# tiiuae/MLAdversarialObjectDetection

Measured on AMD Instinct MI355X. Metric: patch-opt images/sec (EffDet-D0 512px fwd+bwd), higher is better.
Workload: dtype f32; 1 GPU; C2: EfficientDet-D0 patch attack 512x512, 16 images/GPU, bn=local; global_batch=16, image_size=512, placement=injected, parallelism=dp1

## Files before the change

### mladversarialobjectdetection_amd/build.py

```python
import os
import subprocess
import sys

HERE = os.path.dirname(os.path.abspath(__file__))


def build(jobs: int = 8, verbose: bool = False) -> str:
    csrc = os.path.join(HERE, "csrc")
    env = dict(os.environ)
    cmd = ["make", "-C", csrc, f"-j{min(jobs, 16)}"]
    r = subprocess.run(cmd, env=env, stdout=subprocess.PIPE, stderr=subprocess.STDOUT, text=True)
    if verbose or r.returncode != 0:
        sys.stdout.write(r.stdout)
    if r.returncode != 0:
        raise RuntimeError("libphx build failed")
    kern = os.path.join(os.path.dirname(HERE), "tests", "kernels")
    if os.path.isfile(os.path.join(kern, "Makefile")):
        r = subprocess.run(["make", "-C", kern, f"-j{min(jobs, 16)}"], env=env, stdout=subprocess.PIPE,
                           stderr=subprocess.STDOUT, text=True)
        if verbose or r.returncode != 0:
            sys.stdout.write(r.stdout)
        if r.returncode != 0:
            raise RuntimeError("tests/kernels build failed")
    return os.path.join(HERE, "libphx.so")


if __name__ == "__main__":
    print(build(verbose=True))
```

### mladversarialobjectdetection_amd/csrc/api.cpp

```cpp
#include "ctx.hpp"

namespace {

std::string json_escape(const std::string& s) {
  std::string o;
  for (char c : s) {
    if (c == '"' || c == '\\') o.push_back('\\');
    o.push_back(c);
  }
  return o;
}

std::vector<float> make_anchors(const ModelConfig& mc) {
  std::vector<int> fs{mc.image_size};
  int f = mc.image_size;
  for (int l = 1; l <= mc.max_level; ++l) {
    f = (f - 1) / 2 + 1;
    fs.push_back(f);
  }
  std::vector<float> out;
  for (int level = mc.min_level; level <= mc.max_level; ++level) {
    const double stride = (double)fs[0] / (double)fs[level];
    struct C { double base_x, base_y, ax, ay; };
    std::vector<C> cs;
// ... 688 lines not shown
  PHX_CATCH(ctx)
}

int phx_debug_tap(phx_ctx* ctx, const char* op_name, int which, float* out, size_t nfloats, void* stream) {
  if (!ctx || !op_name || !out || ctx->execs.empty()) return PHX_EINVAL;
  PHX_TRY(ctx)
  if (!ctx->last) throw std::logic_error("no step has run");
  Exec& E = *ctx->last;
  for (size_t i = 0; i < E.prog.ops.size(); ++i) {
    const Op& op = E.prog.ops[i];
    if (op.name != op_name) continue;
    const int t = (op.t == OP_BN && which == 0) ? op.in[0] : op.out;
    if (nfloats != E.prog.tensors[t].numel())
      throw std::invalid_argument("tap: size mismatch (the tensor has " + std::to_string(E.prog.tensors[t].numel()) +
                                  " elements)");
    if (which == 0 && op.t == OP_FUSE && E.fuse_folded[i])
      throw std::invalid_argument("tap: this fuse is computed on load by its depthwise conv, never stored");
    if (which == 1 && op.t == OP_DW && E.sepb[i])
      throw std::invalid_argument("tap: this depthwise output's gradient is formed in LDS by the fused "
                                  "separable-conv backward, never stored (PHX_SEPB=0 keeps it)");
    if (which == 0 && op.t == OP_DW && E.sep[i])
      throw std::invalid_argument("tap: this depthwise output feeds the fused separable conv's registers only, "
                                  "never stored (PHX_SEP=0 at victim creation keeps it)");
    const float* src = which == 0 ? E.tptr(t, nullptr) : E.gptr(op.out);
    if (!src) throw std::invalid_argument("tap: no gradient for this tensor");
    if (which == 0 && E.tbf(t)) launch_bf16_to_f32(src, out, (long)nfloats, (hipStream_t)stream);
    else PHX_HIP(hipMemcpyAsync(out, src, nfloats * 4, hipMemcpyDeviceToDevice, (hipStream_t)stream));
    return PHX_OK;
  }
  throw std::invalid_argument(std::string("tap: no op named ") + op_name);
  PHX_CATCH(ctx)
}

int phx_debug_tensor(phx_ctx* ctx, int tag, int op_index, int which, void* out, size_t nbytes, void* stream) {
  if (!ctx || !out || ctx->execs.empty()) return PHX_EINVAL;
  PHX_TRY(ctx)
  if (!ctx->last) throw std::logic_error("no step has run");
  Exec* E = nullptr;
  for (auto& e : ctx->execs)
    if (e->B == ctx->last->B && e->tag == tag) E = e.get();
  if (!E) throw std::invalid_argument("tensor: no executor with this tag");
  if (op_index < 0 || op_index >= (int)E->prog.ops.size() || which < 0 || which > 2)
    throw std::invalid_argument("tensor: bad op index / which");
  const Op& op = E->prog.ops[op_index];
  const int t = which == 0 ? op.out : op.in[which - 1];
  if (t < 0 || t == E->prog.input) throw std::invalid_argument("tensor: no such arena tensor");
// ... 64 lines not shown
```

### mladversarialobjectdetection_amd/csrc/dw_stage.hpp

```cpp
#pragma once
#include <type_traits>

#include "common.hpp"

namespace phx {

__device__ __forceinline__ bool dw_block_map(int L, int per, int ncg, int nwork, int* tile,
                                             int* cg) {
  const int w = (L & 7) * per + (L >> 3);
  if ((L >> 3) >= per || w >= nwork) return false;
  *tile = w / ncg;
  *cg = w - *tile * ncg;
  return true;
}

template <bool BF>
struct StageInX {
  using Raw = float4;
  InX v;
  Chan4 k;
  bool f;
  __device__ __forceinline__ void init(const InX& x, int c) {
    v = x;
    f = x.mu != nullptr;
// ... 68 lines not shown
  }
  __device__ __forceinline__ Raw zero() const {
    return Raw{make_float4(0.f, 0.f, 0.f, 0.f), make_float4(0.f, 0.f, 0.f, 0.f)};
  }
  __device__ __forceinline__ Raw load(long e) const {
    Raw r;
    r.d = *reinterpret_cast<const float4*>(g.da + e);
    if (g.y) r.y = ald4<BF>(g.y, e);
    return r;
  }
  __device__ __forceinline__ float4 finish(const Raw& r) const {
    return g.y ? gx_apply4(g, k, r.d, r.y) : r.d;
  }
  static constexpr bool kActT = true;
  __device__ __forceinline__ int act() const { return g.y ? g.act : 0; }
  template <int ACT>
  __device__ __forceinline__ float4 finish_t(const Raw& r) const {
    GradX c = g;
    c.act = ACT;
    return g.y ? gx_apply4(c, k, r.d, r.y) : r.d;
  }
};

__device__ __forceinline__ void fma4(float4& a, const float4& x, const float4& w) {
  a.x = fmaf(x.x, w.x, a.x);
  a.y = fmaf(x.y, w.y, a.y);
  a.z = fmaf(x.z, w.z, a.z);
  a.w = fmaf(x.w, w.w, a.w);
}

}
```

### mladversarialobjectdetection_amd/csrc/exec.cpp

```cpp
#include "ctx.hpp"

constexpr size_t kMaxExecs = 4;

namespace {

void alloc_exec(Exec& E, int A) {
  const Program& P = E.prog;
  const int B = E.B;
  E.act = E.alloc<float>(E.abf ? (P.act_floats + 1) / 2 : P.act_floats);
  E.grad = E.alloc<float>(E.tag != 0 ? 1 : P.grad_floats);
  E.slot_a.assign(P.n_slots, nullptr);
  E.slot_b.assign(P.n_slots, nullptr);
  E.slot_c.assign(P.n_slots, nullptr);
  E.slot_d.assign(P.n_slots, nullptr);
  E.slot_e.assign(P.n_slots, nullptr);
  for (const Op& op : P.ops) {
    const Tensor& ti = P.tensors[op.in[0]];
    if (op.t == OP_BN) {
      E.slot_a[op.slot] = E.alloc<float>(ti.c);
      E.slot_b[op.slot] = E.alloc<float>(ti.c);
      E.slot_c[op.slot] = E.alloc<float>(ti.c);
      E.slot_d[op.slot] = E.alloc<float>(ti.c);
      E.slot_e[op.slot] = E.alloc<float>(ti.c);
      PHX_HIP(hipMemset(E.slot_d[op.slot], 0, ti.c * sizeof(float)));
// ... 201 lines not shown
  if (op.t == OP_BN) {
    ck_note(E, nm + " mean", E.slot_a[op.slot], ti.c * 4, s);
    ck_note(E, nm + " rstd", E.slot_b[op.slot], ti.c * 4, s);
    ck_note(E, nm + " scale", E.slot_c[op.slot], ti.c * 4, s);
  } else if (op.t == OP_SE) {
    ck_note(E, nm + " excite", E.slot_c[op.slot], (size_t)E.B * ti.c * 4, s);
  } else {
    const Tensor& to = P.tensors[op.out];
    ck_note(E, nm + " out", E.tptr(op.out, nullptr), to.numel() * (E.tbf(op.out) ? 2 : 4), s);
  }
}

void ck_post(Exec& E, int pass, hipStream_t s) {
  const size_t n0 = E.ck_names.size();
  for (size_t i = 0; i < E.prog.ops.size(); ++i) ck_fwd(E, (int)i, pass, s);
  for (size_t k = n0; k < E.ck_names.size(); ++k) E.ck_names[k] = "post " + E.ck_names[k];
}

static void ck_bwd(Exec& E, int i, hipStream_t s) {
  if (!E.ck_on) return;
  const Program& P = E.prog;
  const Op& op = P.ops[i];
  const std::string nm = "b " + std::to_string(i) + " " + op.name;
  if (op.t == OP_BN) {
    const int C = P.tensors[op.in[0]].c;
    ck_note(E, nm + " mdz", E.slot_d[op.slot], C * 4, s);
    ck_note(E, nm + " mdzx", E.slot_e[op.slot], C * 4, s);
    return;
  }
  for (int k = 0; k < op.nin; ++k)
    if (const float* g = E.gptr(op.in[k])) ck_note(E, nm + " d" + std::to_string(k), g, P.tensors[op.in[k]].numel() * 4, s);
}

static bool frozen_reuse_off() {
  return !env_on("PHX_FROZEN_REUSE");
}


static void sync_reduce_apply(phx_ctx* ctx, Exec& E, const BnFinSeg* segs, int n, int C, bool bwd, hipStream_t s) {
  if (!ctx->ar_fn) throw std::logic_error("bn=sync: no collective registered (phx_set_allreduce)");
  if (ctx->ar_fn(ctx->ar_user, E.sync_sums, (size_t)n * C * 3, s) != 0)
    throw std::runtime_error("bn=sync: the all-reduce callback failed");
  launch_bn_from_sums(segs, n, C, bwd, E.sync_sums, kBnEps, s);
}

static void sync_finalize(phx_ctx* ctx, Exec& E, const BnFinSeg* segs, int n, int C, bool bwd, hipStream_t s) {
// ... 503 lines not shown
  else
    for (size_t k = 0; k < zp.size(); ++k) PHX_HIP(hipMemsetAsync(zp[k], 0, zb[k], s));
  launch_cls_scatter(E.scores, E.keep, E.mraw, E.nties, E.dm, E.tptr(P.cls_out[0], input),
                     E.lev_dev, (int)E.lev.size(), ctx->A, E.B, ctx->mc.num_classes, na,
                     W + wpred, K, E.grad, E.dxoff_dev, s, E.tbf(P.cls_out[0]));
  for (int i = (int)P.ops.size() - 1; i >= 0; --i) {
    const Op& op = P.ops[i];
    if (!op.bwd) continue;
    if (op.t == OP_PW && is_cls_out(P, op.out)) continue;
    if (i > 0 && E.sepb[i - 1]) continue;
    if (E.grp_of[i] >= 0) {
      if (E.groups[E.grp_of[i]].back() == i) {
        if (E.sepb[i]) run_sep_bwd(ctx, E, i, input, s);
        else run_group_bwd(ctx, E, E.grp_of[i], input, s);
        for (int m : E.groups[E.grp_of[i]]) ck_bwd(E, m, s);
      }
      continue;
    }
    if (E.sepb[i]) {
      run_sep_bwd(ctx, E, i, input, s);
      ck_bwd(E, i, s);
      continue;
    }
    const Tensor& ti = P.tensors[op.in[0]];
    const Tensor& to = P.tensors[op.out];
    const float* dy = E.gptr(op.out);
    float* dx = E.gptr(op.in[0]);
    double fl = 0, by = 4.0 * (double)(ti.numel() + to.numel());
    const char* kind = "bwd_other";
    switch (op.t) {
      case OP_STEM: kind = "stem_bwd"; fl = 2.0 * to.numel() * 27; break;
      case OP_PW: kind = "gemm"; fl = 2.0 * ti.rows() * ti.c * to.c; by += 4.0 * ti.c * to.c; break;
      case OP_DW: kind = "dw_bwd"; fl = 2.0 * to.numel() * op.k * op.k; break;
      case OP_BN: kind = "bn_bwd_reduce"; by = 4.0 * 2.0 * ti.numel(); break;
      case OP_SE: kind = "se_bwd"; by = 4.0 * 3.0 * ti.numel(); break;
      default: break;
    }
    if (op.t == OP_PW || op.t == OP_DW) {
      const int bi = E.bn_consumer[op.out];
      if (bi >= 0 && P.ops[bi].bwd) by += 4.0 * (double)to.numel();
      if (op.acc[0]) by += 4.0 * (double)ti.numel();
    }
    GradSink gsk{};
    int gsk_in = -1;
    if (i > 0 && E.gfused_bn[i - 1]) {
      const Op& bn = P.ops[i - 1];
      gsk = GradSink{E.spart, P.tensors[bn.out].c, 0, E.tptr(bn.in[0], input), E.slot_a[bn.slot],
                     E.slot_b[bn.slot], E.slot_c[bn.slot], W + bn.beta, bn.act, E.tbf(bn.in[0])};
      gsk_in = op.in[0] == bn.out ? 0 : 1;
    }
    if (op.t == OP_BN && E.gfused_bn[i]) by = 8.0 * (double)E.gstat_P[i] * ti.c;
    if (skip_kind(std::string("b:") + kind, op.name)) continue;
    Scope scope(ctx, kind, fl, by, s, (prof_detail() || debug_sync()) ? op_tag(P, op, true) : std::string());
    int np = -1;
    switch (op.t) {
      case OP_STEM: {
        GradX g = gview(ctx, E, op.out, input);
        if (!op.acc[0] && stem_bwd_gx_supported(to.c)) {
          launch_stem_bwd_gx(g, W + op.w, E.owner, dx, ti.n, ti.h, ti.w, to.h, to.w, to.c, op.pad_t,
                             op.pad_l, s);
          break;
        }
        float* gy = E.gptr(op.out);
        if (g.y) launch_bn_bwd_apply2(g, gy, (long)to.rows(), to.c, s);
        launch_stem_bwd(g.y ? gy : g.da, W + op.w, dx, ti.n, ti.h, ti.w, to.h, to.w, to.c, op.pad_t, op.pad_l,
                        op.acc[0], s);
        break;
      }
      case OP_PW:
        np = launch_gemm_dgrad(gview(ctx, E, op.out, input), W + op.w, dx, (int)ti.rows(), ti.c, to.c,
                               op.acc[0], s, E.gpart, gsk, E.bf16);
        break;
      case OP_DW:
        np = launch_dw_bwd(gview(ctx, E, op.out, input), W + op.w, dx, ti.n, ti.h, ti.w, ti.c, to.h, to.w, op.k,
                           op.stride, op.pad_t, op.pad_l, op.acc[0], s, gsk);
        break;
      case OP_BN:
        if (op.acc[0]) throw std::runtime_error("BN input with several consumers");
        if (!frozen && E.gfused_bn[i] && ctx->bn_mode == PHX_BN_SYNC) {
          const BnFinSeg sg{E.spart + E.gstat_region[i] * E.sp_region, nullptr, E.gstat_P[i], (long)ti.rows(),
                            nullptr, nullptr, nullptr, nullptr, nullptr, nullptr, E.slot_d[op.slot], E.slot_e[op.slot]};
          sync_finalize(ctx, E, &sg, 1, ti.c, true, s);
        } else if (!frozen && E.gfused_bn[i] && skip_timing('b')) {
        } else if (!frozen && E.gfused_bn[i])
          launch_bn_bwd_finalize(E.spart + E.gstat_region[i] * E.sp_region, E.gstat_P[i], (long)ti.rows(),
                                 ti.c, E.slot_d[op.slot],
                                 E.slot_e[op.slot], s);
        else if (!frozen && ctx->bn_mode == PHX_BN_SYNC) {
          launch_bn_bwd_reduce_sums(dy, E.tptr(op.in[0], input), E.slot_a[op.slot], E.slot_b[op.slot], W + op.gamma,
                                    W + op.beta, (long)ti.rows(), ti.c, op.act, E.red, E.sync_sums, s,
                                    E.tbf(op.in[0]) != 0);
          const BnFinSeg sg{nullptr, nullptr, 0, (long)ti.rows(), nullptr, nullptr, nullptr, nullptr, nullptr, nullptr,
                            E.slot_d[op.slot], E.slot_e[op.slot]};
          sync_reduce_apply(ctx, E, &sg, 1, ti.c, true, s);
        }
        else if (!frozen)
          launch_bn_bwd_reduce(dy, E.tptr(op.in[0], input), E.slot_a[op.slot], E.slot_b[op.slot],
                               W + op.gamma, W + op.beta, (long)ti.rows(), ti.c, op.act, E.red,
                               E.slot_d[op.slot], E.slot_e[op.slot], s, E.tbf(op.in[0]) != 0);
        (void)dx;
        break;
      case OP_SE:
        np = launch_se_bwd(dy, view(ctx, E, op.in[0], input), dx, ti.n, ti.h * ti.w, ti.c, op.cse, W + op.w1,
                           W + op.b1, ctx->wt_of(op.w2), W + op.b2, op.act, E.slot_a[op.slot],
                           E.slot_b[op.slot], E.slot_c[op.slot], E.se_g, op.acc[0], s, E.red, gsk);
        break;
      case OP_ADD: {
        int n0 = 0, n1 = 0;
        if (dx == dy) {
          if (gsk_in == 0) n0 = launch_grad_sums(dy, (long)to.numel(), to.c, gsk, s);
        } else {
          n0 = launch_copy_grad(dy, dx, (long)to.numel(), op.acc[0], s, to.c,
                                gsk_in == 0 ? gsk : GradSink{}, drop_view(E, i));
        }
        if (E.gptr(op.in[1]) == dy) {
          if (gsk_in == 1) n1 = launch_grad_sums(dy, (long)to.numel(), to.c, gsk, s);
        } else {
          n1 = launch_copy_grad(dy, E.gptr(op.in[1]), (long)to.numel(), op.acc[1], s, to.c,
                                gsk_in == 1 ? gsk : GradSink{});
        }
        np = gsk_in == 0 ? n0 : n1;
        break;
      }
      case OP_MAXPOOL:
        launch_maxpool_bwd(E.pool_amax[i], dy, dx, ti.n, ti.h, ti.w, ti.c, to.h, to.w,
// ... 106 lines not shown
```

### mladversarialobjectdetection_amd/csrc/exec_plan.cpp

```cpp
#include "exec_plan.hpp"

#include <algorithm>
#include <map>
#include <stdexcept>

#include "env.hpp"
#include "phx.h"

namespace phx {

bool is_cls_out(const Program& P, int t) {
  return std::find(P.cls_out.begin(), P.cls_out.end(), t) != P.cls_out.end();
}

namespace {

bool grouping_enabled() {
  static const bool on = env_on("PHX_GROUP");
  return on;
}

bool group_uniform(const ExecPlan& E, const std::vector<int>& v) {
  const Program& P = E.prog;
  const Op& a = P.ops[v[0]];
// ... 264 lines not shown
      if (gd >= 0 && E.groups[gd][0] != (int)i) continue;
      const std::vector<int> mem = gd >= 0 ? E.groups[gd] : std::vector<int>{(int)i};
      bool ok = true;
      for (int di : mem) {
        const Op& d = P.ops[di];
        const Op& pw = P.ops[di + 1];
        const int bi = E.bn_consumer[pw.out];
        ok = ok && d.bwd && pw.bwd && !is_cls_out(P, pw.out) && bi >= 0 && P.ops[bi].bwd &&
             sep_bwd_supported(P.tensors[d.in[0]].c, P.tensors[pw.out].c, E.bf16 || E.abf);
        ok = ok && (di > 0 && E.gfused_bn[di - 1]) == (mem[0] > 0 && E.gfused_bn[mem[0] - 1]);
      }
      if (!ok) continue;
      for (int di : mem) {
        E.sepb[di] = 1;
        if (di > 0 && E.gfused_bn[di - 1]) {
          const Tensor& tm = P.tensors[P.ops[di].in[0]];
          const int np = sep_stat_partials(tm.n, tm.h, tm.w);
          E.gstat_P[di - 1] = np;
          sp_need = std::max(sp_need, (size_t)np * tm.c);
        }
      }
    }
  }
  E.nreg = E.groups.empty() ? 1 : kMaxSeg;
  E.sp_region = sp_need;
  E.sc_region = sc_need;
  for (const Op& op : P.ops) {
    if (op.t != OP_PW) continue;
    const Tensor& ti = P.tensors[op.in[0]];
    const Tensor& to = P.tensors[op.out];
    E.gp_need = std::max(E.gp_need, gemm_partial_floats((int)ti.rows(), to.c, ti.c, bf16));
    E.gp_need = std::max(E.gp_need, gemm_partial_floats((int)ti.rows(), ti.c, to.c, bf16));
  }
  const int nlev = (int)P.cls_out.size();
  int a0 = 0;
  for (int l = 0; l < nlev; ++l) {
    const Tensor& tc = P.tensors[P.cls_out[l]];
    const Tensor& tb = P.tensors[P.box_out[l]];
    LevelDesc d;
    d.cls_off = (long)tc.off - (long)P.tensors[P.cls_out[0]].off;
    d.box_off = (long)tb.off - (long)P.tensors[P.box_out[0]].off;
    d.h = tc.h;
    d.w = tc.w;
    d.anchor0 = a0;
    d.tile0 = E.ntiles;
    E.ntiles += pre_nms_tiles(tc.h, tc.w, na);
// ... 27 lines not shown
```

### mladversarialobjectdetection_amd/csrc/exec_plan.hpp

```cpp
#pragma once
#include <vector>

#include "common.hpp"
#include "kernels.hpp"
#include "model.hpp"
#include "post.hpp"

namespace phx {

struct ExecPlan {
  Program prog;
  int B = 0;
  int tag = 0;
  bool bf16 = false;
  bool abf = false;
  bool infer_plan = false;
  std::vector<int> se_of_tensor;
  std::vector<int> bn_of_tensor;
  std::vector<int> bn_consumer;
  std::vector<char> fused_bn;
  std::vector<char> gfused_bn;
  std::vector<int> gstat_P;
  std::vector<int> grp_of;
  std::vector<std::vector<int>> groups;
  std::vector<char> fuse_folded;
  std::vector<char> sep;
  std::vector<char> sepb;
  std::vector<int> drop_slot;
  std::vector<int> side_off;
  std::vector<MovEntry> mov;
  int n_mov = 0, mov_cmax = 1;
  std::vector<LevelDesc> lev;
  std::vector<long> dxoff;
  int ntiles = 0;
  int ndrop = 0;
  std::vector<int> drop_blocks;
  std::vector<float> drop_surv;
  EotDims ed{};
  size_t red_need = 1, coef_need = 1, seg_need = 1, gp_need = 1;
  size_t sp_region = 1, sc_region = 1, nreg = 1;
  size_t side_need = 2, sync_need = 0;
};

ExecPlan plan_exec(const ModelConfig& mc, int B, int tag, int bn_mode, bool bf16, int num_anchors);

ExecPlan plan_program(const Program& prog, int B, int tag, int bn_mode, bool bf16, int image_size, int na,
                      int num_anchors);

bool is_cls_out(const Program& P, int t);

// ... 2 lines not shown
```

### mladversarialobjectdetection_amd/csrc/kernels.hpp

```cpp
#pragma once
#include <hip/hip_runtime.h>
#include <hip/hip_ext.h>

#include <cstddef>
#include <cstdint>

#include "common.hpp"

namespace phx {

struct ExtTiming {
  hipEvent_t a = nullptr, b = nullptr;
  bool used = false;
};
ExtTiming*& ext_timing();
#define PHX_TLAUNCH(K, G, BL, SHM, S, ...)                                                              \
  do {                                                                                                 \
    if (::phx::ExtTiming* t_ = ::phx::ext_timing()) {                                                  \
      hipExtLaunchKernelGGL(K, G, BL, SHM, S, t_->used ? nullptr : t_->a, t_->b, 0, __VA_ARGS__);      \
      t_->used = true;                                                                                 \
    } else {                                                                                           \
      hipLaunchKernelGGL(K, G, BL, SHM, S, __VA_ARGS__);                                               \
    }                                                                                                  \
  } while (0)
// ... 49 lines not shown
int gemm_dgrad_gsink_partials(int M, int N, int K, bool bf16 = false);
bool gemm_fold_ok(int M, int N, int K, bool bf16);
struct GemmSeg {
  InX A;
  GradX G;
  const float* bias;
  float* C;
  int M;
  bool acc;
  StatSink sink;
  GradSink gsk;
};
bool gemm_group_ok(const int* M, int n, int N, int K, bool bf16 = false);
int gemm_group_run(int mode, const GemmSeg* segs, int n, const float* Bt, int N, int K, hipStream_t s,
                   bool bf16 = false, int* P_out = nullptr, long max_part_rows = -1);
int launch_dw_fwd(InX x, const float* w, float* y, int B, int H, int W, int C, int Ho,
                  int Wo, int k, int stride, int pt, int pl, hipStream_t s,
                  StatSink sink = StatSink{});
int dw_stat_partials(int B, int H, int W, int C, int Ho, int Wo, int k, int stride, int pt, int pl);
int launch_dw_bwd(GradX dy, const float* w, float* dx, int B, int H, int W, int C, int Ho,
                  int Wo, int k, int stride, int pt, int pl, bool acc, hipStream_t s,
                  GradSink gs = GradSink{});
int dw_bwd_partials(int B, int H, int W, int C, int Ho, int Wo, int k, int stride, int pt, int pl);
struct DwSeg {
  InX x;
  GradX gv;
  float* out;
  int H, W, Ho, Wo, pt, pl;
  bool acc;
  StatSink sink;
  GradSink gs;
};
void launch_dw_fwd_group(const DwSeg* segs, int n, int B, int C, const float* w, int k, int stride,
                         hipStream_t s, int* nps);
struct SepMember {
  InX x;
  FuseView f;
  bool fuse;
  float* y;
  int H, W;
  StatSink sink;
};
bool sep_supported(int C, int N, bool bf16);
int sep_stat_partials(int B, int H, int W);
void launch_sep_fwd(const SepMember* m, int n, int B, int C, int N, const float* wd, const float* bt,
                    const float* bias, hipStream_t s, int* nps);
// ... 64 lines not shown
void launch_bn_stats_sums(const float* y, long M, int C, double* part, double* sums, hipStream_t s, bool ybf);
void launch_bn_bwd_reduce_sums(const float* da, const float* y, const float* mean, const float* rstd,
                               const float* gamma, const float* beta, long M, int C, int act, double* part,
                               double* sums, hipStream_t s, bool ybf);
void launch_bn_bwd_finalize_group(const BnFinSeg* segs, int n, int C, hipStream_t s);
void launch_bn_frozen_stats(const float* mmean, const float* mvar, float* mean, float* rstd,
                            const float* gamma, float* sc, int C, float eps, hipStream_t s);
void launch_bn_apply(const float* y, const float* mean, const float* rstd, const float* gamma,
                     const float* beta, float* a, long M, int C, int act, hipStream_t s);
void launch_bn_bwd(const float* da, const float* y, const float* mean, const float* rstd,
                   const float* gamma, const float* beta, float* dy, long M, int C, int act,
                   bool frozen, bool acc, double* part, float* coef, hipStream_t s);
void launch_bn_bwd_apply2(GradX g, float* out, long M, int C, hipStream_t s);
void launch_bn_bwd_reduce(const float* da, const float* y, const float* mean, const float* rstd,
                          const float* gamma, const float* beta, long M, int C, int act,
                          double* part, float* mdz, float* mdzx, hipStream_t s, bool ybf = false);
void launch_se_fwd(InX x, float* y, int B, int HW, int C, int Cse, const float* w1,
                   const float* b1, const float* w2, const float* b2, int act, float* pool,
                   float* hidden, float* scale, hipStream_t s, double* scratch);
int launch_se_bwd(const float* dy, InX x, float* dx, int B, int HW, int C, int Cse,
                  const float* w1, const float* b1, const float* w2t, const float* b2, int act,
                  const float* pool, const float* hidden, const float* scale, float* gsum,
                  bool acc, hipStream_t s, double* scratch, GradSink gs = GradSink{});
int ew_gstats_partials(long seg_rows, int C, int nseg);
void launch_bn_bwd_finalize(const float2* part, int P, long M, int C, float* mdz, float* mdzx,
                            hipStream_t s);
size_t colred_scratch_doubles(long seg_rows, int C, int nseg);
struct RedPlanInfo {
  int tpr, rpi, cgroups, chunks, tpr_last, depth;
  long rpc;
};
RedPlanInfo red_plan_info(long seg_rows, int C, int nseg);
struct SePlanInfo {
  int s1, cs1, s2, cs2, fold_small, kg, jg;
};
SePlanInfo se_plan_info(int B, int C, int Cse, int chunks);
struct DropView {
  const float* keep = nullptr;
  float p = 1.f;
  long rows = 1;
};
void launch_drop_keep(const int* block, const float* p, int nd, int B, uint64_t seed, int64_t step,
                      int gimg0, int pass, float* keep, hipStream_t s);
void launch_bf16_to_f32(const float* src, float* dst, long n, hipStream_t s);
void launch_cksum(const void* p, size_t bytes, unsigned long long* out, hipStream_t s);
void launch_add(InX a, InX b, float* y, long n, int C, hipStream_t s, DropView dv = DropView{});
// ... 87 lines not shown
```

### mladversarialobjectdetection_amd/csrc/kernels_dw.hip

```cpp
#include <algorithm>
#include <cstdlib>
#include <stdexcept>
#include <type_traits>

#include "env.hpp"
#include "dw_stage.hpp"
#include "kernels.hpp"

namespace phx {

struct DwGeom {
  int H, W, C;
  int Ho, Wo;
  int pt, pl;
  int lcg;
  int otw, oth;
  int nrg;
  int rin, cin;
  int tiles_x, ntiles, ncg;
  int per;
};

template <class XV>
struct DwFwdSegT {
  XV x;
  float* y;
  DwGeom g;
  StatSink sink;
};
using DwFwdSeg = DwFwdSegT<InX>;
template <int NS, class XV = InX>
struct DwFwdGroup {
  DwFwdSegT<XV> s[NS];
  const float* w;
};
struct DwBwdSeg {
  GradX gv;
  float* dx;
  DwGeom g;
  int acc;
  GradSink gs;
};
template <int NS>
struct DwBwdGroup {
  DwBwdSeg s[NS];
  const float* w;
};

#ifndef PHX_DW_LDS_TAPS
#define PHX_DW_LDS_TAPS 2
#endif
template <int K>
struct Taps {
  static constexpr bool kLds = PHX_DW_LDS_TAPS == 2 || (PHX_DW_LDS_TAPS == 1 && K > 3);
  float4 r[kLds ? 1 : K * K];
  const float4* l;
  int cg, CG;
  __device__ __forceinline__ void stage(float4* wt, const float* w, int C, int cgi, int lcg) {
    if constexpr (kLds) {
      const int n = (K * K) << lcg;
      for (int e = threadIdx.x; e < n; e += 256) {
        const int t = e >> lcg, k = e & ((1 << lcg) - 1);
        wt[e] = *reinterpret_cast<const float4*>(w + (long)t * C + (((cgi << lcg) + k) << 2));
      }
// ... 190 lines not shown
  const int lane = threadIdx.x & 63, wave = threadIdx.x >> 6;
  s1 = dw_xor_sum(s1, lcg);
  s2 = dw_xor_sum(s2, lcg);
  if (lane < CG) {
    a_[wave][cg] = s1;
    b_[wave][cg] = s2;
  }
  __syncthreads();
  if (threadIdx.x < CG) {
    float4 t1 = a_[0][cg], t2 = b_[0][cg];
#pragma unroll
    for (int w = 1; w < 4; ++w) {
      const float4 u = a_[w][cg], v = b_[w][cg];
      t1.x += u.x; t1.y += u.y; t1.z += u.z; t1.w += u.w;
      t2.x += v.x; t2.y += v.y; t2.z += v.z; t2.w += v.w;
    }
    gsink_put(g, p, c + 0, t1.x, t2.x);
    gsink_put(g, p, c + 1, t1.y, t2.y);
    gsink_put(g, p, c + 2, t1.z, t2.z);
    gsink_put(g, p, c + 3, t1.w, t2.w);
  }
}

template <int K, int S, int RPT, bool GS, int NS, int SU = 4, bool YBF = false>
__global__ __launch_bounds__(256) void k_dw_bwd(DwBwdGroup<NS> grp) {
  const DwBwdSeg sg = pick_seg(grp.s, NS == 1 ? 0 : (int)blockIdx.y);
  const GradX& gv = sg.gv;
  const DwGeom& g = sg.g;
  const GradSink& gsk = sg.gs;
  const int acc_flag = sg.acc;
  const float* __restrict__ w = grp.w;
  float* __restrict__ dx = sg.dx;
  extern __shared__ float4 tile[];
  const int b = blockIdx.z;
  int tl, cgi;
  if (!dw_block_map(blockIdx.x, g.per, g.ncg, g.ntiles * g.ncg, &tl, &cgi)) return;
  const int CG = 1 << g.lcg;
  const int ty = tl / g.tiles_x, tx = tl - ty * g.tiles_x;
  const int iy0 = ty * g.oth, ix0 = tx * g.otw;
  const int cg = threadIdx.x & (CG - 1), q = threadIdx.x >> g.lcg;
  const int col = q % g.otw, rg = q / g.otw;
  const int c = (cgi * CG + cg) * 4;
  const int ay = iy0 + g.pt - (K - 1), ax = ix0 + g.pl - (K - 1);
  const int oy_lo = S == 1 ? ay : (ay >= 0 ? ay / S : -((-ay + S - 1) / S));
  const int ox_lo = S == 1 ? ax : (ax >= 0 ? ax / S : -((-ax + S - 1) / S));

  StageGradX<YBF> src;
  src.init(gv, c);
  float4* wt = tile + g.rin * g.cin * CG;
  Taps<K> wr;
  wr.stage(wt, w, g.C, cgi, g.lcg);
  dw_stage<StageGradX<YBF>, SU>(tile, src, b, g.Ho, g.Wo, g.C, oy_lo, ox_lo, c, g);
  __syncthreads();

  const int ix = ix0 + col;
  const int row0 = rg * RPT;
  const bool active = rg < g.nrg && ix < g.W && iy0 + row0 < g.H;
  if (!GS && !active) return;
  float4 acc[RPT];
#pragma unroll
  for (int r = 0; r < RPT; ++r) acc[r] = make_float4(0.f, 0.f, 0.f, 0.f);
  if (active) {
    wr.init(wt, w, g.C, c, cg, g.lcg);
    if constexpr (S == 1) {
      constexpr int NR = RPT + K - 1;
      const float4* base = tile + (row0 * g.cin + col) * CG + cg;
#pragma unroll
      for (int ir = 0; ir < NR; ++ir) {
#pragma unroll
        for (int jj = 0; jj < K; ++jj) {
          const float4 v = base[(ir * g.cin + jj) * CG];
#pragma unroll
          for (int r = 0; r < RPT; ++r) {
            const int ii = ir - r;
            if (ii >= 0 && ii < K) fma4(acc[r], v, wr((K - 1 - ii) * K + (K - 1 - jj)));
// ... 180 lines not shown
  if (dw_lds(grp.s[0].g, k) > 160 * 1024) throw std::runtime_error("dw: LDS window too large");
  dw_fwd_go<3, 1, 4, 1, FuseView>(grp, 1, B, false, s);
  PHX_LAUNCH_CHECK();
}

void launch_dw_fwd_group(const DwSeg* segs, int n, int B, int C, const float* w, int k, int stride,
                         hipStream_t s, int* nps) {
  if (C % 4) throw std::runtime_error("dw: C % 4 != 0");
  if (n < 1 || n > kMaxSeg) throw std::runtime_error("dw group: bad member count");
  const int rpt = dw_rpt_fwd(stride);
  DwFwdGroup<kMaxSeg> grp{};
  grp.w = w;
  const bool stats = segs[0].sink.part != nullptr;
  for (int i = 0; i < n; ++i) {
    const DwSeg& d = segs[i];
    if ((d.sink.part != nullptr) != stats) throw std::runtime_error("dw group: members differ in sinks");
    grp.s[i] = DwFwdSeg{d.x, d.out, dw_plan(d.H, d.W, C, d.Ho, d.Wo, d.pt, d.pl, k, stride, rpt, false), d.sink};
    grp.s[i].sink.P = B * grp.s[i].g.ntiles;
    nps[i] = grp.s[i].sink.P;
  }
  dw_fwd_dispatch(grp, n, B, stats, k, stride, s);
}

template <int K, int S, int NS>
static void dw_bwd_go(const DwBwdGroup<NS>& grp, int n, int B, bool gsums, hipStream_t s) {
  int gx = 1;
  size_t lds = 0;
  for (int i = 0; i < n; ++i) {
    gx = std::max(gx, 8 * grp.s[i].g.per);
    lds = std::max(lds, dw_lds(grp.s[i].g, K));
  }
  dim3 grid(gx, n, B);
  const bool ybf = (grp.s[0].gv.y && grp.s[0].gv.ybf) || (gsums && grp.s[0].gs.ybf);
  if (ybf) {
    if (gsums)
      hipLaunchKernelGGL((k_dw_bwd<K, S, 4, true, NS, 4, true>), grid, dim3(256), lds, s, grp);
    else
      hipLaunchKernelGGL((k_dw_bwd<K, S, 4, false, NS, 4, true>), grid, dim3(256), lds, s, grp);
    return;
  }
  if (gsums)
    hipLaunchKernelGGL((k_dw_bwd<K, S, 4, true, NS>), grid, dim3(256), lds, s, grp);
  else
    hipLaunchKernelGGL((k_dw_bwd<K, S, 4, false, NS>), grid, dim3(256), lds, s, grp);
}

template <int NS>
static void dw_bwd_dispatch(const DwBwdGroup<NS>& grp, int n, int B, bool gsums, int k, int stride,
                            hipStream_t s) {
  for (int i = 0; i < n; ++i)
    if (dw_lds(grp.s[i].g, k) > 160 * 1024) throw std::runtime_error("dw: LDS window too large");
  if (k == 3 && stride == 1) dw_bwd_go<3, 1, NS>(grp, n, B, gsums, s);
  else if (k == 3 && stride == 2) dw_bwd_go<3, 2, NS>(grp, n, B, gsums, s);
  else if (k == 5 && stride == 1) dw_bwd_go<5, 1, NS>(grp, n, B, gsums, s);
  else if (k == 5 && stride == 2) dw_bwd_go<5, 2, NS>(grp, n, B, gsums, s);
  else throw std::invalid_argument("dw: unsupported kernel/stride");
  PHX_LAUNCH_CHECK();
}

int dw_bwd_partials(int B, int H, int W, int C, int Ho, int Wo, int k, int stride, int pt, int pl) {
  DwGeom g = dw_plan(H, W, C, Ho, Wo, pt, pl, k, stride, 4, true);
  return B * g.ntiles;
}

int launch_dw_bwd(GradX dy, const float* w, float* dx, int B, int H, int W, int C, int Ho,
                  int Wo, int k, int stride, int pt, int pl, bool acc, hipStream_t s, GradSink gs) {
  if (C % 4) throw std::runtime_error("dw: C % 4 != 0");
  DwBwdGroup<1> grp{};
  grp.w = w;
  grp.s[0] = DwBwdSeg{dy, dx, dw_plan(H, W, C, Ho, Wo, pt, pl, k, stride, 4, true), acc ? 1 : 0, gs};
  grp.s[0].gs.P = B * grp.s[0].g.ntiles;
  dw_bwd_dispatch(grp, 1, B, gs.part != nullptr, k, stride, s);
  return B * grp.s[0].g.ntiles;
}

void launch_dw_bwd_group(const DwSeg* segs, int n, int B, int C, const float* w, int k, int stride,
                         hipStream_t s, int* nps) {
  if (C % 4) throw std::runtime_error("dw: C % 4 != 0");
  if (n < 1 || n > kMaxSeg) throw std::runtime_error("dw group: bad member count");
  DwBwdGroup<kMaxSeg> grp{};
  grp.w = w;
  const bool gsums = segs[0].gs.part != nullptr;
  for (int i = 0; i < n; ++i) {
    const DwSeg& d = segs[i];
    if ((d.gs.part != nullptr) != gsums) throw std::runtime_error("dw group: members differ in sinks");
    grp.s[i] = DwBwdSeg{d.gv, d.out, dw_plan(d.H, d.W, C, d.Ho, d.Wo, d.pt, d.pl, k, stride, 4, true),
                        d.acc ? 1 : 0, d.gs};
    grp.s[i].gs.P = B * grp.s[i].g.ntiles;
    nps[i] = grp.s[i].gs.P;
  }
  dw_bwd_dispatch(grp, n, B, gsums, k, stride, s);
}

static DwTileInfo dw_info_of(const DwGeom& g, int rpt) {
  return DwTileInfo{g.lcg, rpt, g.otw, g.oth, g.nrg, g.rin, g.cin, g.tiles_x, g.ntiles, g.ncg, 0, 0};
// ... 18 lines not shown
```

### mladversarialobjectdetection_amd/csrc/kernels_norm.hip

```cpp
#include <algorithm>
#include <cstdlib>

#include "common.hpp"
#include "env.hpp"
#include "kernels.hpp"

namespace phx {

struct RedPlan {
  int tpr;
  int cgroups;
  int chunks;
  long rpc;
};

static long red_target_blocks() {
  static long v = env_long("PHX_RED_BLOCKS", 1024L);
  return v;
}
static int red_depth() {
  static int v = [] {
    const char* e = std::getenv("PHX_RED_DEPTH");
    return (e && atoi(e) == 4) ? 4 : 8;
  }();
// ... 921 lines not shown
  __device__ float4 out(const Raw& g, long m, int c4) const {
    float4 o = make_float4(fmaf(g.x, sc.x, dp.x), fmaf(g.y, sc.y, dp.y), fmaf(g.z, sc.z, dp.z), fmaf(g.w, sc.w, dp.w));
    float4* op = reinterpret_cast<float4*>(dx + m * C + c4 * 4);
    if (acc) {
      const float4 p = *op;
      o.x += p.x; o.y += p.y; o.z += p.z; o.w += p.w;
    }
    *op = o;
    return o;
  }
};

int launch_se_bwd(const float* dy, InX x, float* dx, int B, int HW, int C, int Cse,
                  const float* w1, const float* b1, const float* w2t, const float* b2, int act,
                  const float* pool, const float* hidden, const float* scale, float* gsum,
                  bool acc, hipStream_t s, double* scratch, GradSink gs) {
  if (Cse < 1 || Cse > kSeT) throw std::runtime_error("se: squeeze width outside 1..256");
  (void)b1; (void)b2; (void)pool;
  const int chunks = x.bf ? colred_parts(SumAcc<true>{x, dy, C, {}}, HW, C, B, scratch, s)
                          : colred_parts(SumAcc<false>{x, dy, C, {}}, HW, C, B, scratch, s);
  se_mlp<1>(scratch, chunks, B, C, Cse, 1.f, w2t, nullptr, w1, nullptr, act, scale, nullptr,
            const_cast<float*>(hidden), gsum, s);
  return ew_gstats(SeBwdApply{dy, scale, gsum, dx, C, acc ? 1 : 0, 1.0f / (float)HW, {}, {}}, HW, C, B, gs, s);
}

__device__ __forceinline__ float4 drop_fwd4(const DropView& dv, long row, float4 u) {
  const float k = dv.keep[row / dv.rows];
  return make_float4(div_surv(u.x, dv.p) * k, div_surv(u.y, dv.p) * k, div_surv(u.z, dv.p) * k,
                     div_surv(u.w, dv.p) * k);
}
__device__ __forceinline__ float4 drop_bwd4(const DropView& dv, long row, float4 g) {
  const float k = dv.keep[row / dv.rows];
  return make_float4(div_surv(g.x * k, dv.p), div_surv(g.y * k, dv.p), div_surv(g.z * k, dv.p),
                     div_surv(g.w * k, dv.p));
}

template <bool BF>
__global__ void k_add(InX a, InX b, float* __restrict__ y, long n4, int C, DropView dv) {
  long i = (long)blockIdx.x * blockDim.x + threadIdx.x;
  if (i >= n4) return;
  const int c = (int)((i * 4) % C);
  float4 u = inx_load4<BF>(a, i * 4, c), v = inx_load4<BF>(b, i * 4, c);
  if (dv.keep) u = drop_fwd4(dv, i * 4 / C, u);
  ast4<BF>(y, i * 4, make_float4(u.x + v.x, u.y + v.y, u.z + v.z, u.w + v.w));
}

// ... 549 lines not shown
```

Measured before the change: 1458 images/s.

## Fold SE backward apply into depthwise-conv backward input staging

```diff
diff --git a/mladversarialobjectdetection_amd/build.py b/mladversarialobjectdetection_amd/build.py
--- a/mladversarialobjectdetection_amd/build.py
+++ b/mladversarialobjectdetection_amd/build.py
@@ -14,14 +14,16 @@
         sys.stdout.write(r.stdout)
     if r.returncode != 0:
         raise RuntimeError("libphx build failed")
-    kern = os.path.join(os.path.dirname(HERE), "tests", "kernels")
-    if os.path.isfile(os.path.join(kern, "Makefile")):
+    for sub in ("kernels", "kernels_sefold"):
+        kern = os.path.join(os.path.dirname(HERE), "tests", sub)
+        if not os.path.isfile(os.path.join(kern, "Makefile")):
+            continue
         r = subprocess.run(["make", "-C", kern, f"-j{min(jobs, 16)}"], env=env, stdout=subprocess.PIPE,
                            stderr=subprocess.STDOUT, text=True)
         if verbose or r.returncode != 0:
             sys.stdout.write(r.stdout)
         if r.returncode != 0:
-            raise RuntimeError("tests/kernels build failed")
+            raise RuntimeError(f"tests/{sub} build failed")
     return os.path.join(HERE, "libphx.so")
 
 
diff --git a/mladversarialobjectdetection_amd/csrc/api.cpp b/mladversarialobjectdetection_amd/csrc/api.cpp
--- a/mladversarialobjectdetection_amd/csrc/api.cpp
+++ b/mladversarialobjectdetection_amd/csrc/api.cpp
@@ -734,6 +734,14 @@
     if (which == 0 && op.t == OP_DW && E.sep[i])
       throw std::invalid_argument("tap: this depthwise output feeds the fused separable conv's registers only, "
                                   "never stored (PHX_SEP=0 at victim creation keeps it)");
+    if (which == 1 && op.t == OP_BN && i + 1 < E.prog.ops.size() && E.sefold[i + 1]) {
+      const Op& se = E.prog.ops[i + 1];
+      const Tensor& tb = E.prog.tensors[op.out];
+      if (!E.gptr(se.out)) throw std::invalid_argument("tap: no gradient for this tensor");
+      launch_se_da(E.gptr(se.out), E.slot_c[se.slot], E.gptr(op.out), out, tb.n, tb.h * tb.w, tb.c,
+                   (hipStream_t)stream);
+      return PHX_OK;
+    }
     const float* src = which == 0 ? E.tptr(t, nullptr) : E.gptr(op.out);
     if (!src) throw std::invalid_argument("tap: no gradient for this tensor");
     if (which == 0 && E.tbf(t)) launch_bf16_to_f32(src, out, (long)nfloats, (hipStream_t)stream);
diff --git a/mladversarialobjectdetection_amd/csrc/dw_stage.hpp b/mladversarialobjectdetection_amd/csrc/dw_stage.hpp
--- a/mladversarialobjectdetection_amd/csrc/dw_stage.hpp
+++ b/mladversarialobjectdetection_amd/csrc/dw_stage.hpp
@@ -114,6 +114,33 @@
   }
 };
 
+template <bool BF>
+struct StageGradXSe {
+  using Raw = typename StageGradX<BF>::Raw;
+  StageGradX<BF> x;
+  float4 s, q;
+  __device__ __forceinline__ void init(const GradX& gx, const float* sp, const float* dp, float inv, int C, int b,
+                                       int c) {
+    x.init(gx, c);
+    s = *reinterpret_cast<const float4*>(sp + (long)b * C + c);
+    const float4 d = *reinterpret_cast<const float4*>(dp + (long)b * C + c);
+    q = make_float4(d.x * inv, d.y * inv, d.z * inv, d.w * inv);
+  }
+  __device__ __forceinline__ Raw zero() const { return x.zero(); }
+  __device__ __forceinline__ Raw load(long e) const { return x.load(e); }
+  __device__ __forceinline__ Raw se(const Raw& r) const {
+    return Raw{make_float4(fmaf(r.d.x, s.x, q.x), fmaf(r.d.y, s.y, q.y), fmaf(r.d.z, s.z, q.z), fmaf(r.d.w, s.w, q.w)),
+               r.y};
+  }
+  __device__ __forceinline__ float4 finish(const Raw& r) const { return x.finish(se(r)); }
+  static constexpr bool kActT = true;
+  __device__ __forceinline__ int act() const { return x.act(); }
+  template <int ACT>
+  __device__ __forceinline__ float4 finish_t(const Raw& r) const {
+    return x.template finish_t<ACT>(se(r));
+  }
+};
+
 __device__ __forceinline__ void fma4(float4& a, const float4& x, const float4& w) {
   a.x = fmaf(x.x, w.x, a.x);
   a.y = fmaf(x.y, w.y, a.y);
diff --git a/mladversarialobjectdetection_amd/csrc/exec.cpp b/mladversarialobjectdetection_amd/csrc/exec.cpp
--- a/mladversarialobjectdetection_amd/csrc/exec.cpp
+++ b/mladversarialobjectdetection_amd/csrc/exec.cpp
@@ -247,6 +247,11 @@
   const Program& P = E.prog;
   const Op& op = P.ops[i];
   const std::string nm = "b " + std::to_string(i) + " " + op.name;
+  if (op.t == OP_SE && E.sefold[i]) {
+    const Tensor& ti = P.tensors[op.in[0]];
+    ck_note(E, nm + " dpool", E.gptr(op.in[0]), (size_t)ti.n * ti.c * 4, s);
+    return;
+  }
   if (op.t == OP_BN) {
     const int C = P.tensors[op.in[0]].c;
     ck_note(E, nm + " mdz", E.slot_d[op.slot], C * 4, s);
@@ -796,6 +801,8 @@
       ck_bwd(E, i, s);
       continue;
     }
+    const bool se_fold = op.t == OP_SE && E.sefold[i];
+    const bool dw_fold = op.t == OP_DW && i + 2 < (int)P.ops.size() && E.sefold[i + 2];
     const Tensor& ti = P.tensors[op.in[0]];
     const Tensor& to = P.tensors[op.out];
     const float* dy = E.gptr(op.out);
@@ -807,7 +814,7 @@
       case OP_PW: kind = "gemm"; fl = 2.0 * ti.rows() * ti.c * to.c; by += 4.0 * ti.c * to.c; break;
       case OP_DW: kind = "dw_bwd"; fl = 2.0 * to.numel() * op.k * op.k; break;
       case OP_BN: kind = "bn_bwd_reduce"; by = 4.0 * 2.0 * ti.numel(); break;
-      case OP_SE: kind = "se_bwd"; by = 4.0 * 3.0 * ti.numel(); break;
+      case OP_SE: kind = "se_bwd"; by = 4.0 * (se_fold ? 2.0 : 3.0) * ti.numel(); break;
       default: break;
     }
     if (op.t == OP_PW || op.t == OP_DW) {
@@ -846,6 +853,15 @@
                                op.acc[0], s, E.gpart, gsk, E.bf16);
         break;
       case OP_DW:
+        if (dw_fold) {
+          const Op& se = P.ops[i + 2];
+          const Tensor& tb = P.tensors[se.in[0]];
+          GradX g = gview(ctx, E, op.out, input);
+          g.da = E.gptr(se.out);
+          np = launch_dw_bwd_se(g, E.slot_c[se.slot], E.gptr(se.in[0]), 1.0f / (float)(tb.h * tb.w), W + op.w, dx, ti.n, ti.h, ti.w, ti.c, to.h, to.w, op.k, op.stride, op.pad_t, op.pad_l,
+                                op.acc[0], s, gsk);
+          break;
+        }
         np = launch_dw_bwd(gview(ctx, E, op.out, input), W + op.w, dx, ti.n, ti.h, ti.w, ti.c, to.h, to.w, op.k,
                            op.stride, op.pad_t, op.pad_l, op.acc[0], s, gsk);
         break;
@@ -875,6 +891,11 @@
         (void)dx;
         break;
       case OP_SE:
+        if (se_fold) {
+          np = launch_se_bwd_sums(dy, view(ctx, E, op.in[0], input), ti.n, ti.h * ti.w, ti.c, op.cse, W + op.w1,
+                                  ctx->wt_of(op.w2), op.act, E.slot_b[op.slot], E.slot_c[op.slot], dx, s, E.red, gsk);
+          break;
+        }
         np = launch_se_bwd(dy, view(ctx, E, op.in[0], input), dx, ti.n, ti.h * ti.w, ti.c, op.cse, W + op.w1,
                            W + op.b1, ctx->wt_of(op.w2), W + op.b2, op.act, E.slot_a[op.slot],
                            E.slot_b[op.slot], E.slot_c[op.slot], E.se_g, op.acc[0], s, E.red, gsk);
diff --git a/mladversarialobjectdetection_amd/csrc/exec_plan.cpp b/mladversarialobjectdetection_amd/csrc/exec_plan.cpp
--- a/mladversarialobjectdetection_amd/csrc/exec_plan.cpp
+++ b/mladversarialobjectdetection_amd/csrc/exec_plan.cpp
@@ -310,6 +310,20 @@
       }
     }
   }
+  E.sefold.assign(P.ops.size(), 0);
+  {
+    const bool on = env_on("PHX_SEFOLD") && bbn && bn_mode == PHX_BN_LOCAL;
+    for (size_t i = 2; on && i < P.ops.size(); ++i) {
+      const Op& se = P.ops[i];
+      const Op& bn = P.ops[i - 1];
+      const Op& dw = P.ops[i - 2];
+      if (se.t != OP_SE || !se.bwd || se.acc[0]) continue;
+      if (bn.t != OP_BN || !bn.bwd || bn.out != se.in[0] || !E.gfused_bn[i - 1] || E.grp_of[i - 1] >= 0) continue;
+      if (dw.t != OP_DW || !dw.bwd || dw.out != bn.in[0] || E.grp_of[i - 2] >= 0 || E.sepb[i - 2]) continue;
+      if (P.tensors[se.in[0]].c % 4 || P.tensors[se.in[0]].goff < 0) continue;
+      E.sefold[i] = 1;
+    }
+  }
   E.nreg = E.groups.empty() ? 1 : kMaxSeg;
   E.sp_region = sp_need;
   E.sc_region = sc_need;
diff --git a/mladversarialobjectdetection_amd/csrc/exec_plan.hpp b/mladversarialobjectdetection_amd/csrc/exec_plan.hpp
--- a/mladversarialobjectdetection_amd/csrc/exec_plan.hpp
+++ b/mladversarialobjectdetection_amd/csrc/exec_plan.hpp
@@ -26,6 +26,7 @@
   std::vector<char> fuse_folded;
   std::vector<char> sep;
   std::vector<char> sepb;
+  std::vector<char> sefold;
   std::vector<int> drop_slot;
   std::vector<int> side_off;
   std::vector<MovEntry> mov;
diff --git a/mladversarialobjectdetection_amd/csrc/kernels.hpp b/mladversarialobjectdetection_amd/csrc/kernels.hpp
--- a/mladversarialobjectdetection_amd/csrc/kernels.hpp
+++ b/mladversarialobjectdetection_amd/csrc/kernels.hpp
@@ -95,6 +95,9 @@
                   int Wo, int k, int stride, int pt, int pl, bool acc, hipStream_t s,
                   GradSink gs = GradSink{});
 int dw_bwd_partials(int B, int H, int W, int C, int Ho, int Wo, int k, int stride, int pt, int pl);
+int launch_dw_bwd_se(GradX dy, const float* se_s, const float* se_dpool, float se_inv, const float* w, float* dx,
+                     int B, int H, int W, int C, int Ho, int Wo, int k, int stride, int pt, int pl, bool acc,
+                     hipStream_t s, GradSink gs = GradSink{});
 struct DwSeg {
   InX x;
   GradX gv;
@@ -205,6 +208,11 @@
                   const float* w1, const float* b1, const float* w2t, const float* b2, int act,
                   const float* pool, const float* hidden, const float* scale, float* gsum,
                   bool acc, hipStream_t s, double* scratch, GradSink gs = GradSink{});
+int launch_se_bwd_sums(const float* dy, InX x, int B, int HW, int C, int Cse, const float* w1, const float* w2t,
+                       int act, const float* hidden, const float* scale, float* dpool, hipStream_t s,
+                       double* scratch, GradSink gs);
+void launch_se_da(const float* dy, const float* scale, const float* dpool, float* out, int B, int HW, int C,
+                  hipStream_t s);
 int ew_gstats_partials(long seg_rows, int C, int nseg);
 void launch_bn_bwd_finalize(const float2* part, int P, long M, int C, float* mdz, float* mdzx,
                             hipStream_t s);
diff --git a/mladversarialobjectdetection_amd/csrc/kernels_dw.hip b/mladversarialobjectdetection_amd/csrc/kernels_dw.hip
--- a/mladversarialobjectdetection_amd/csrc/kernels_dw.hip
+++ b/mladversarialobjectdetection_amd/csrc/kernels_dw.hip
@@ -40,6 +40,9 @@
   DwGeom g;
   int acc;
   GradSink gs;
+  const float* se_s = nullptr;
+  const float* se_d = nullptr;
+  float se_inv = 0.f;
 };
 template <int NS>
 struct DwBwdGroup {
@@ -276,7 +279,7 @@
   }
 }
 
-template <int K, int S, int RPT, bool GS, int NS, int SU = 4, bool YBF = false>
+template <int K, int S, int RPT, bool GS, int NS, int SU = 4, bool YBF = false, bool SE = false>
 __global__ __launch_bounds__(256) void k_dw_bwd(DwBwdGroup<NS> grp) {
   const DwBwdSeg sg = pick_seg(grp.s, NS == 1 ? 0 : (int)blockIdx.y);
   const GradX& gv = sg.gv;
@@ -299,12 +302,14 @@
   const int oy_lo = S == 1 ? ay : (ay >= 0 ? ay / S : -((-ay + S - 1) / S));
   const int ox_lo = S == 1 ? ax : (ax >= 0 ? ax / S : -((-ax + S - 1) / S));
 
-  StageGradX<YBF> src;
-  src.init(gv, c);
+  using Stage = std::conditional_t<SE, StageGradXSe<YBF>, StageGradX<YBF>>;
+  Stage src;
+  if constexpr (SE) src.init(gv, sg.se_s, sg.se_d, sg.se_inv, g.C, b, c);
+  else src.init(gv, c);
   float4* wt = tile + g.rin * g.cin * CG;
   Taps<K> wr;
   wr.stage(wt, w, g.C, cgi, g.lcg);
-  dw_stage<StageGradX<YBF>, SU>(tile, src, b, g.Ho, g.Wo, g.C, oy_lo, ox_lo, c, g);
+  dw_stage<Stage, SU>(tile, src, b, g.Ho, g.Wo, g.C, oy_lo, ox_lo, c, g);
   __syncthreads();
 
   const int ix = ix0 + col;
@@ -531,7 +536,7 @@
   dw_fwd_dispatch(grp, n, B, stats, k, stride, s);
 }
 
-template <int K, int S, int NS>
+template <int K, int S, int NS, bool SE = false>
 static void dw_bwd_go(const DwBwdGroup<NS>& grp, int n, int B, bool gsums, hipStream_t s) {
   int gx = 1;
   size_t lds = 0;
@@ -543,26 +548,26 @@
   const bool ybf = (grp.s[0].gv.y && grp.s[0].gv.ybf) || (gsums && grp.s[0].gs.ybf);
   if (ybf) {
     if (gsums)
-      hipLaunchKernelGGL((k_dw_bwd<K, S, 4, true, NS, 4, true>), grid, dim3(256), lds, s, grp);
+      hipLaunchKernelGGL((k_dw_bwd<K, S, 4, true, NS, 4, true, SE>), grid, dim3(256), lds, s, grp);
     else
-      hipLaunchKernelGGL((k_dw_bwd<K, S, 4, false, NS, 4, true>), grid, dim3(256), lds, s, grp);
+      hipLaunchKernelGGL((k_dw_bwd<K, S, 4, false, NS, 4, true, SE>), grid, dim3(256), lds, s, grp);
     return;
   }
   if (gsums)
-    hipLaunchKernelGGL((k_dw_bwd<K, S, 4, true, NS>), grid, dim3(256), lds, s, grp);
+    hipLaunchKernelGGL((k_dw_bwd<K, S, 4, true, NS, 4, false, SE>), grid, dim3(256), lds, s, grp);
   else
-    hipLaunchKernelGGL((k_dw_bwd<K, S, 4, false, NS>), grid, dim3(256), lds, s, grp);
-}
-
-template <int NS>
+    hipLaunchKernelGGL((k_dw_bwd<K, S, 4, false, NS, 4, false, SE>), grid, dim3(256), lds, s, grp);
+}
+
+template <int NS, bool SE = false>
 static void dw_bwd_dispatch(const DwBwdGroup<NS>& grp, int n, int B, bool gsums, int k, int stride,
                             hipStream_t s) {
   for (int i = 0; i < n; ++i)
     if (dw_lds(grp.s[i].g, k) > 160 * 1024) throw std::runtime_error("dw: LDS window too large");
-  if (k == 3 && stride == 1) dw_bwd_go<3, 1, NS>(grp, n, B, gsums, s);
-  else if (k == 3 && stride == 2) dw_bwd_go<3, 2, NS>(grp, n, B, gsums, s);
-  else if (k == 5 && stride == 1) dw_bwd_go<5, 1, NS>(grp, n, B, gsums, s);
-  else if (k == 5 && stride == 2) dw_bwd_go<5, 2, NS>(grp, n, B, gsums, s);
+  if (k == 3 && stride == 1) dw_bwd_go<3, 1, NS, SE>(grp, n, B, gsums, s);
+  else if (k == 3 && stride == 2) dw_bwd_go<3, 2, NS, SE>(grp, n, B, gsums, s);
+  else if (k == 5 && stride == 1) dw_bwd_go<5, 1, NS, SE>(grp, n, B, gsums, s);
+  else if (k == 5 && stride == 2) dw_bwd_go<5, 2, NS, SE>(grp, n, B, gsums, s);
   else throw std::invalid_argument("dw: unsupported kernel/stride");
   PHX_LAUNCH_CHECK();
 }
@@ -580,6 +585,21 @@
   grp.s[0] = DwBwdSeg{dy, dx, dw_plan(H, W, C, Ho, Wo, pt, pl, k, stride, 4, true), acc ? 1 : 0, gs};
   grp.s[0].gs.P = B * grp.s[0].g.ntiles;
   dw_bwd_dispatch(grp, 1, B, gs.part != nullptr, k, stride, s);
+  return B * grp.s[0].g.ntiles;
+}
+
+int launch_dw_bwd_se(GradX dy, const float* se_s, const float* se_dpool, float se_inv, const float* w, float* dx,
+                     int B, int H, int W, int C, int Ho, int Wo, int k, int stride, int pt, int pl, bool acc,
+                     hipStream_t s, GradSink gs) {
+  if (C % 4) throw std::runtime_error("dw: C % 4 != 0");
+  if (!dy.y || !se_s || !se_dpool) throw std::runtime_error("dw bwd se: needs a BN gradient view, s and dpool");
+  if ((reinterpret_cast<uintptr_t>(se_s) | reinterpret_cast<uintptr_t>(se_dpool)) & 15)
+    throw std::runtime_error("dw bwd se: unaligned s / dpool");
+  DwBwdGroup<1> grp{};
+  grp.w = w;
+  grp.s[0] = DwBwdSeg{dy, dx, dw_plan(H, W, C, Ho, Wo, pt, pl, k, stride, 4, true), acc ? 1 : 0, gs, se_s, se_dpool, se_inv};
+  grp.s[0].gs.P = B * grp.s[0].g.ntiles;
+  dw_bwd_dispatch<1, true>(grp, 1, B, gs.part != nullptr, k, stride, s);
   return B * grp.s[0].g.ntiles;
 }
 
diff --git a/mladversarialobjectdetection_amd/csrc/kernels_norm.hip b/mladversarialobjectdetection_amd/csrc/kernels_norm.hip
--- a/mladversarialobjectdetection_amd/csrc/kernels_norm.hip
+++ b/mladversarialobjectdetection_amd/csrc/kernels_norm.hip
@@ -967,6 +967,61 @@
   se_mlp<1>(scratch, chunks, B, C, Cse, 1.f, w2t, nullptr, w1, nullptr, act, scale, nullptr,
             const_cast<float*>(hidden), gsum, s);
   return ew_gstats(SeBwdApply{dy, scale, gsum, dx, C, acc ? 1 : 0, 1.0f / (float)HW, {}, {}}, HW, C, B, gs, s);
+}
+
+struct SeBwdSums {
+  const float* dy;
+  const float* scale;
+  const float* dpool;
+  int C;
+  float inv;
+  float4 sc, dp;
+  using Raw = float4;
+  __device__ void init(int seg, int c4) {
+    sc = *reinterpret_cast<const float4*>(scale + (long)seg * C + c4 * 4);
+    const float4 d = *reinterpret_cast<const float4*>(dpool + (long)seg * C + c4 * 4);
+    dp = make_float4(d.x * inv, d.y * inv, d.z * inv, d.w * inv);
+  }
+  __device__ Raw load(long m, int c4) const { return *reinterpret_cast<const float4*>(dy + m * C + c4 * 4); }
+  __device__ float4 out(const Raw& g, long, int) const {
+    return make_float4(fmaf(g.x, sc.x, dp.x), fmaf(g.y, sc.y, dp.y), fmaf(g.z, sc.z, dp.z), fmaf(g.w, sc.w, dp.w));
+  }
+};
+
+int launch_se_bwd_sums(const float* dy, InX x, int B, int HW, int C, int Cse, const float* w1, const float* w2t,
+                       int act, const float* hidden, const float* scale, float* dpool, hipStream_t s,
+                       double* scratch, GradSink gs) {
+  if (Cse < 1 || Cse > kSeT) throw std::runtime_error("se: squeeze width outside 1..256");
+  if (!gs.part) throw std::runtime_error("se bwd sums: no GradSink (nothing else is produced)");
+  if (reinterpret_cast<uintptr_t>(dpool) & 15) throw std::runtime_error("se bwd sums: unaligned dpool");
+  const int chunks = x.bf ? colred_parts(SumAcc<true>{x, dy, C, {}}, HW, C, B, scratch, s)
+                          : colred_parts(SumAcc<false>{x, dy, C, {}}, HW, C, B, scratch, s);
+  se_mlp<1>(scratch, chunks, B, C, Cse, 1.f, w2t, nullptr, w1, nullptr, act, scale, nullptr,
+            const_cast<float*>(hidden), dpool, s);
+  return ew_gstats(SeBwdSums{dy, scale, dpool, C, 1.0f / (float)HW, {}, {}}, HW, C, B, gs, s);
+}
+
+__global__ __launch_bounds__(256) void k_se_da(const float4* __restrict__ dy, const float* __restrict__ scale,
+                                               const float* __restrict__ dpool, float inv, float4* __restrict__ out,
+                                               long n4, long per_img, int C) {
+  const long i = (long)blockIdx.x * blockDim.x + threadIdx.x;
+  if (i >= n4) return;
+  const long e = i * 4;
+  const long bc = (e / per_img) * C + e % C;
+  const float4 g = dy[i];
+  const float4 sc = *reinterpret_cast<const float4*>(scale + bc);
+  const float4 d = *reinterpret_cast<const float4*>(dpool + bc);
+  out[i] = make_float4(fmaf(g.x, sc.x, d.x * inv), fmaf(g.y, sc.y, d.y * inv), fmaf(g.z, sc.z, d.z * inv),
+                       fmaf(g.w, sc.w, d.w * inv));
+}
+
+void launch_se_da(const float* dy, const float* scale, const float* dpool, float* out, int B, int HW, int C,
+                  hipStream_t s) {
+  if (C % 4) throw std::runtime_error("se da: C % 4 != 0");
+  const long n4 = (long)B * HW * C / 4;
+  hipLaunchKernelGGL(k_se_da, dim3(cdiv(n4, 256)), dim3(256), 0, s, reinterpret_cast<const float4*>(dy), scale, dpool,
+                     1.0f / (float)HW, reinterpret_cast<float4*>(out), n4, (long)HW * C, C);
+  PHX_LAUNCH_CHECK();
 }
 
 __device__ __forceinline__ float4 drop_fwd4(const DropView& dv, long row, float4 u) {
```

New measurement: 1479 images/s (median of 6 runs). 1.4% higher.
